# leggedrobotics/wild_visual_navigation

Hardware: NVIDIA H100
Metric: frames/sec end-to-end (DINO feat + seg + MLP train-step) at 448x448 (higher is better)
Workload: dtype bf16 operands / fp32 accumulate (ViT, STEGO head, per-pixel MLP); fp32 (k-means, train step)

## Files before the change

wild_visual_navigation_b200/csrc/common.cuh:

```cuda
#pragma once

#include <cuda.h>
#include <cuda_bf16.h>
#include <cuda_runtime.h>
#include <stdint.h>
#include <stdio.h>

namespace wvn {

__device__ __forceinline__ uint32_t smem_u32(const void* p) {
  return static_cast<uint32_t>(__cvta_generic_to_shared(p));
}

__device__ __forceinline__ bool elect_one_sync() {
  uint32_t pred;
  asm volatile(
      "{\n\t"
      ".reg .pred p;\n\t"
      "elect.sync _|p, 0xffffffff;\n\t"
      "selp.u32 %0, 1, 0, p;\n\t"
      "}"
      : "=r"(pred));
  return pred != 0;
}

__device__ __forceinline__ uint32_t pack_bf16x2(float lo, float hi) {
  __nv_bfloat162 v = __floats2bfloat162_rn(lo, hi);
  return *reinterpret_cast<uint32_t*>(&v);
}

__device__ __forceinline__ float bf16_lo(uint32_t v) { return __uint_as_float(v << 16); }
__device__ __forceinline__ float bf16_hi(uint32_t v) { return __uint_as_float(v & 0xffff0000u); }

__device__ __forceinline__ void mbar_init(uint64_t* bar, uint32_t count) {
  asm volatile("mbarrier.init.shared::cta.b64 [%0], %1;" ::"r"(smem_u32(bar)), "r"(count) : "memory");
}

__device__ __forceinline__ void fence_mbar_init() {
  asm volatile("fence.mbarrier_init.release.cluster;" ::: "memory");
}

__device__ __forceinline__ void mbar_arrive_expect_tx(uint64_t* bar, uint32_t bytes) {
  asm volatile("mbarrier.arrive.expect_tx.shared::cta.b64 _, [%0], %1;" ::"r"(smem_u32(bar)), "r"(bytes)
               : "memory");
}

__device__ __forceinline__ void mbar_arrive(uint64_t* bar) {
  asm volatile("mbarrier.arrive.shared::cta.b64 _, [%0];" ::"r"(smem_u32(bar)) : "memory");
}

__device__ __forceinline__ bool mbar_try_wait(uint64_t* bar, uint32_t parity) {
  uint32_t ok;
  asm volatile(
      "{\n\t"
      ".reg .pred p;\n\t"
      "mbarrier.try_wait.parity.shared::cta.b64 p, [%1], %2;\n\t"
      "selp.u32 %0, 1, 0, p;\n\t"
      "}"
      : "=r"(ok)
      : "r"(smem_u32(bar)), "r"(parity)
      : "memory");
  return ok != 0;
}

__device__ __forceinline__ bool mbar_test_wait(uint64_t* bar, uint32_t parity) {
  uint32_t ok;
  asm volatile(
      "{\n\t"
      ".reg .pred p;\n\t"
      "mbarrier.test_wait.parity.shared::cta.b64 p, [%1], %2;\n\t"
      "selp.u32 %0, 1, 0, p;\n\t"
      "}"
      : "=r"(ok)
      : "r"(smem_u32(bar)), "r"(parity)
      : "memory");
  return ok != 0;
}

#ifndef WVN_MBAR_TIMEOUT_CYCLES
#define WVN_MBAR_TIMEOUT_CYCLES 4000000000ll
#endif

#ifndef WVN_MBAR_HINT_NS
#define WVN_MBAR_HINT_NS 0
#endif
#define WVN_STR2(x) #x
#define WVN_STR(x) WVN_STR2(x)
#if WVN_MBAR_HINT_NS > 0
#define WVN_TRY_WAIT_PTX "mbarrier.try_wait.parity.shared::cta.b64 p, [%1], %2, " WVN_STR(WVN_MBAR_HINT_NS) ";\n\t"
#else
#define WVN_TRY_WAIT_PTX "mbarrier.try_wait.parity.shared::cta.b64 p, [%1], %2;\n\t"
#endif

__device__ __forceinline__ bool mbar_try_wait_many(uint32_t bar_addr, uint32_t parity) {
  uint32_t ok;
  asm volatile(
      "{\n\t"
      ".reg .pred p;\n\t"
      ".reg .u32 n;\n\t"
      "mov.u32 n, 65536;\n\t"
      "WVN_WAIT_LOOP:\n\t"
      WVN_TRY_WAIT_PTX
      "@p bra WVN_WAIT_DONE;\n\t"
      "sub.u32 n, n, 1;\n\t"
      "setp.ne.u32 p, n, 0;\n\t"
      "@p bra WVN_WAIT_LOOP;\n\t"
      "WVN_WAIT_DONE:\n\t"
      "selp.u32 %0, 1, 0, p;\n\t"
      "}"
      : "=r"(ok)
      : "r"(bar_addr), "r"(parity)
      : "memory");
  return ok != 0;
}

__device__ __forceinline__ void mbar_wait(uint64_t* bar, uint32_t parity) {
  if (mbar_try_wait(bar, parity)) return;
  const uint32_t addr = smem_u32(bar);
  const long long t0 = clock64();
  while (!mbar_try_wait_many(addr, parity)) {
    if (clock64() - t0 > WVN_MBAR_TIMEOUT_CYCLES) {
#ifdef WVN_MBAR_DIAG
      printf("[wvn] mbarrier timeout: block (%d,%d) thread %d bar@%u parity %u\n", blockIdx.x, blockIdx.y,
             threadIdx.x, addr, parity);
#endif
      __trap();
    }
  }
}

__device__ __forceinline__ void fence_proxy_async_smem() {
  asm volatile("fence.proxy.async.shared::cta;" ::: "memory");
}

__device__ __forceinline__ void tma_load_2d(const CUtensorMap* map, uint64_t* bar, void* smem_dst, int32_t c0,
                                            int32_t c1) {
  asm volatile(
      "cp.async.bulk.tensor.2d.shared::cluster.global.mbarrier::complete_tx::bytes [%0], [%1, {%3, %4}], [%2];" ::"r"(
          smem_u32(smem_dst)),
      "l"(reinterpret_cast<uint64_t>(map)), "r"(smem_u32(bar)), "r"(c0), "r"(c1)
      : "memory");
}

__device__ __forceinline__ void tma_load_2d_mcast(const CUtensorMap* map, uint64_t* bar, void* smem_dst, int32_t c0,
                                                  int32_t c1, uint16_t cta_mask) {
  asm volatile(
      "cp.async.bulk.tensor.2d.shared::cluster.global.mbarrier::complete_tx::bytes.multicast::cluster"
      " [%0], [%1, {%4, %5}], [%2], %3;" ::"r"(smem_u32(smem_dst)),
      "l"(reinterpret_cast<uint64_t>(map)), "r"(smem_u32(bar)), "h"(cta_mask), "r"(c0), "r"(c1)
      : "memory");
}

__device__ __forceinline__ void tma_store_2d(const CUtensorMap* map, const void* smem_src, int32_t c0, int32_t c1) {
  asm volatile("cp.async.bulk.tensor.2d.global.shared::cta.bulk_group [%0, {%2, %3}], [%1];" ::"l"(
                   reinterpret_cast<uint64_t>(map)),
               "r"(smem_u32(smem_src)), "r"(c0), "r"(c1)
               : "memory");
}
__device__ __forceinline__ void tma_reduce_add_2d(const CUtensorMap* map, const void* smem_src, int32_t c0, int32_t c1) {
  asm volatile("cp.reduce.async.bulk.tensor.2d.global.shared::cta.add.bulk_group [%0, {%2, %3}], [%1];" ::"l"(
                   reinterpret_cast<uint64_t>(map)),
               "r"(smem_u32(smem_src)), "r"(c0), "r"(c1)
               : "memory");
}
__device__ __forceinline__ void tma_store_commit() { asm volatile("cp.async.bulk.commit_group;" ::: "memory"); }
template <int N>
__device__ __forceinline__ void tma_store_wait_read() {
  asm volatile("cp.async.bulk.wait_group.read %0;" ::"n"(N) : "memory");
}
template <int N>
__device__ __forceinline__ void tma_store_wait_all() {
  asm volatile("cp.async.bulk.wait_group %0;" ::"n"(N) : "memory");
}

__device__ __forceinline__ uint32_t cluster_ctarank() {
  uint32_t r;
  asm volatile("mov.u32 %0, %%cluster_ctarank;" : "=r"(r));
  return r;
}

__device__ __forceinline__ void cluster_sync_all() {
  asm volatile("barrier.cluster.arrive.release.aligned;" ::: "memory");
  asm volatile("barrier.cluster.wait.acquire.aligned;" ::: "memory");
}

__device__ __forceinline__ void tma_prefetch_desc(const CUtensorMap* map) {
  asm volatile("prefetch.tensormap [%0];" ::"l"(reinterpret_cast<uint64_t>(map)) : "memory");
}

__device__ __forceinline__ uint64_t make_sw128_kmajor_desc(uint32_t smem_addr) {
  uint64_t d = 0;
  d |= static_cast<uint64_t>((smem_addr & 0x3ffff) >> 4);
  d |= static_cast<uint64_t>(1) << 16;
  d |= static_cast<uint64_t>(1024 >> 4) << 32;
  d |= static_cast<uint64_t>(1) << 62;
  return d;
}

__device__ __forceinline__ void wgmma_fence() { asm volatile("wgmma.fence.sync.aligned;" ::: "memory"); }
__device__ __forceinline__ void wgmma_commit() { asm volatile("wgmma.commit_group.sync.aligned;" ::: "memory"); }
template <int N>
__device__ __forceinline__ void wgmma_wait() {
  asm volatile("wgmma.wait_group.sync.aligned %0;" ::"n"(N) : "memory");
}

template <int N>
__device__ __forceinline__ void wgmma_fence_regs(float (&d)[N]) {
#pragma unroll
  for (int i = 0; i < N; ++i) asm volatile("" : "+f"(d[i])::"memory");
}
template <int N>
__device__ __forceinline__ void wgmma_fence_regs(uint32_t (&a)[N]) {
#pragma unroll
  for (int i = 0; i < N; ++i) asm volatile("" : "+r"(a[i])::"memory");
}

template <int N>
__device__ __forceinline__ void setmaxnreg_inc() { asm volatile("setmaxnreg.inc.sync.aligned.u32 %0;" ::"n"(N)); }
template <int N>
__device__ __forceinline__ void setmaxnreg_dec() { asm volatile("setmaxnreg.dec.sync.aligned.u32 %0;" ::"n"(N)); }

__device__ __forceinline__ void wgmma_m64n32k16_ss(float (&d)[16], uint64_t desc_a, uint64_t desc_b, uint32_t accumulate) {
  asm volatile(
      "{\n\t"
      ".reg .pred p;\n\t"
      "setp.ne.b32 p, %18, 0;\n\t"
      "wgmma.mma_async.sync.aligned.m64n32k16.f32.bf16.bf16 "
      "{%0, %1, %2, %3, %4, %5, %6, %7, %8, %9, %10, %11, %12, %13, %14, %15}, "
      "%16, %17, p, 1, 1, 0, 0;\n\t"
      "}"
      : "+f"(d[0]), "+f"(d[1]), "+f"(d[2]), "+f"(d[3]), "+f"(d[4]), "+f"(d[5]), "+f"(d[6]), "+f"(d[7]),
        "+f"(d[8]), "+f"(d[9]), "+f"(d[10]), "+f"(d[11]), "+f"(d[12]), "+f"(d[13]), "+f"(d[14]), "+f"(d[15])
      : "l"(desc_a), "l"(desc_b), "r"(accumulate));
}

__device__ __forceinline__ void wgmma_m64n64k16_ss(float (&d)[32], uint64_t desc_a, uint64_t desc_b, uint32_t accumulate) {
  asm volatile(
      "{\n\t"
      ".reg .pred p;\n\t"
      "setp.ne.b32 p, %34, 0;\n\t"
      "wgmma.mma_async.sync.aligned.m64n64k16.f32.bf16.bf16 "
      "{%0, %1, %2, %3, %4, %5, %6, %7, %8, %9, %10, %11, %12, %13, %14, %15, %16, %17, %18, %19, %20, "
      "%21, %22, %23, %24, %25, %26, %27, %28, %29, %30, %31}, "
      "%32, %33, p, 1, 1, 0, 0;\n\t"
      "}"
      : "+f"(d[0]), "+f"(d[1]), "+f"(d[2]), "+f"(d[3]), "+f"(d[4]), "+f"(d[5]), "+f"(d[6]), "+f"(d[7]),
        "+f"(d[8]), "+f"(d[9]), "+f"(d[10]), "+f"(d[11]), "+f"(d[12]), "+f"(d[13]), "+f"(d[14]), "+f"(d[15]),
        "+f"(d[16]), "+f"(d[17]), "+f"(d[18]), "+f"(d[19]), "+f"(d[20]), "+f"(d[21]), "+f"(d[22]), "+f"(d[23]),
        "+f"(d[24]), "+f"(d[25]), "+f"(d[26]), "+f"(d[27]), "+f"(d[28]), "+f"(d[29]), "+f"(d[30]), "+f"(d[31])
      : "l"(desc_a), "l"(desc_b), "r"(accumulate));
}

__device__ __forceinline__ void wgmma_m64n128k16_ss(float (&d)[64], uint64_t desc_a, uint64_t desc_b, uint32_t accumulate) {
  asm volatile(
      "{\n\t"
      ".reg .pred p;\n\t"
      "setp.ne.b32 p, %66, 0;\n\t"
      "wgmma.mma_async.sync.aligned.m64n128k16.f32.bf16.bf16 "
      "{%0, %1, %2, %3, %4, %5, %6, %7, %8, %9, %10, %11, %12, %13, %14, %15, %16, %17, %18, %19, %20, "
      "%21, %22, %23, %24, %25, %26, %27, %28, %29, %30, %31, %32, %33, %34, %35, %36, %37, %38, %39, "
      "%40, %41, %42, %43, %44, %45, %46, %47, %48, %49, %50, %51, %52, %53, %54, %55, %56, %57, %58, "
      "%59, %60, %61, %62, %63}, "
      "%64, %65, p, 1, 1, 0, 0;\n\t"
      "}"
      : "+f"(d[0]), "+f"(d[1]), "+f"(d[2]), "+f"(d[3]), "+f"(d[4]), "+f"(d[5]), "+f"(d[6]), "+f"(d[7]),
        "+f"(d[8]), "+f"(d[9]), "+f"(d[10]), "+f"(d[11]), "+f"(d[12]), "+f"(d[13]), "+f"(d[14]), "+f"(d[15]),
        "+f"(d[16]), "+f"(d[17]), "+f"(d[18]), "+f"(d[19]), "+f"(d[20]), "+f"(d[21]), "+f"(d[22]), "+f"(d[23]),
        "+f"(d[24]), "+f"(d[25]), "+f"(d[26]), "+f"(d[27]), "+f"(d[28]), "+f"(d[29]), "+f"(d[30]), "+f"(d[31]),
        "+f"(d[32]), "+f"(d[33]), "+f"(d[34]), "+f"(d[35]), "+f"(d[36]), "+f"(d[37]), "+f"(d[38]), "+f"(d[39]),
        "+f"(d[40]), "+f"(d[41]), "+f"(d[42]), "+f"(d[43]), "+f"(d[44]), "+f"(d[45]), "+f"(d[46]), "+f"(d[47]),
        "+f"(d[48]), "+f"(d[49]), "+f"(d[50]), "+f"(d[51]), "+f"(d[52]), "+f"(d[53]), "+f"(d[54]), "+f"(d[55]),
        "+f"(d[56]), "+f"(d[57]), "+f"(d[58]), "+f"(d[59]), "+f"(d[60]), "+f"(d[61]), "+f"(d[62]), "+f"(d[63])
      : "l"(desc_a), "l"(desc_b), "r"(accumulate));
}

__device__ __forceinline__ void wgmma_m64n64k16_rs(float (&d)[32], uint32_t a0, uint32_t a1, uint32_t a2, uint32_t a3,
                                                   uint64_t desc_b, uint32_t accumulate) {
  asm volatile(
      "{\n\t"
      ".reg .pred p;\n\t"
      "setp.ne.b32 p, %37, 0;\n\t"
      "wgmma.mma_async.sync.aligned.m64n64k16.f32.bf16.bf16 "
      "{%0, %1, %2, %3, %4, %5, %6, %7, %8, %9, %10, %11, %12, %13, %14, %15, %16, %17, %18, %19, %20, "
      "%21, %22, %23, %24, %25, %26, %27, %28, %29, %30, %31}, "
      "{%32, %33, %34, %35}, %36, p, 1, 1, 0;\n\t"
      "}"
      : "+f"(d[0]), "+f"(d[1]), "+f"(d[2]), "+f"(d[3]), "+f"(d[4]), "+f"(d[5]), "+f"(d[6]), "+f"(d[7]),
        "+f"(d[8]), "+f"(d[9]), "+f"(d[10]), "+f"(d[11]), "+f"(d[12]), "+f"(d[13]), "+f"(d[14]), "+f"(d[15]),
        "+f"(d[16]), "+f"(d[17]), "+f"(d[18]), "+f"(d[19]), "+f"(d[20]), "+f"(d[21]), "+f"(d[22]), "+f"(d[23]),
        "+f"(d[24]), "+f"(d[25]), "+f"(d[26]), "+f"(d[27]), "+f"(d[28]), "+f"(d[29]), "+f"(d[30]), "+f"(d[31])
      : "r"(a0), "r"(a1), "r"(a2), "r"(a3), "l"(desc_b), "r"(accumulate));
}

__device__ __forceinline__ void named_bar_sync(int id, int nthreads) {
  asm volatile("bar.sync %0, %1;" ::"r"(id), "r"(nthreads) : "memory");
}
__device__ __forceinline__ void named_bar_arrive(int id, int nthreads) {
  asm volatile("bar.arrive %0, %1;" ::"r"(id), "r"(nthreads) : "memory");
}

__device__ __forceinline__ void sts128(uint32_t addr, uint32_t a, uint32_t b, uint32_t c, uint32_t d) {
  asm volatile("st.shared.v4.b32 [%0], {%1, %2, %3, %4};" ::"r"(addr), "r"(a), "r"(b), "r"(c), "r"(d) : "memory");
}
__device__ __forceinline__ uint4 lds128(uint32_t addr) {
  uint4 v;
  asm volatile("ld.shared.v4.b32 {%0, %1, %2, %3}, [%4];" : "=r"(v.x), "=r"(v.y), "=r"(v.z), "=r"(v.w) : "r"(addr) : "memory");
  return v;
}

__device__ __forceinline__ void st_global_v4(void* p, uint32_t a, uint32_t b, uint32_t c, uint32_t d) {
  asm volatile("st.global.v4.b32 [%0], {%1, %2, %3, %4};" ::"l"(p), "r"(a), "r"(b), "r"(c), "r"(d) : "memory");
}

__device__ __forceinline__ float warp_sum(float v) {
#pragma unroll
  for (int o = 16; o > 0; o >>= 1) v += __shfl_xor_sync(0xffffffffu, v, o);
  return v;
}

__device__ __forceinline__ float warp_max(float v) {
#pragma unroll
  for (int o = 16; o > 0; o >>= 1) v = fmaxf(v, __shfl_xor_sync(0xffffffffu, v, o));
  return v;
}

}
```

wild_visual_navigation_b200/csrc/gemm_wgmma.cu:

```cuda
#include <stdlib.h>

#include <algorithm>

#include "common.cuh"
#include "gemm.h"
#include "host_common.h"

namespace wvn {

namespace {

constexpr int BM = 128;
constexpr int BK = 64;
constexpr int kConsumerWarps = 8;
constexpr int kNumThreads = 128 + kConsumerWarps * 32;
constexpr int kMaxSmemBytes = 227 * 1024;
constexpr int kMaxStages = 8;
constexpr int kFixedSmemBytes = 1024  + 1024 ;

template <bool ROW_OWNER>
struct TileIter {
  int num_m, num_n, m_blk, n_blk, lin;
  __device__ TileIter(int nm, int nn) : num_m(nm), num_n(nn), m_blk(0), n_blk(0), lin(0) {
    if (ROW_OWNER) { m_blk = blockIdx.x; n_blk = 0; }
    else { lin = blockIdx.x; m_blk = lin / num_n; n_blk = lin % num_n; }
  }
  __device__ bool valid() const { return m_blk < num_m; }
  __device__ void next() {
    if (ROW_OWNER) { if (++n_blk == num_n) { n_blk = 0; m_blk += gridDim.x; } }
    else { lin += gridDim.x; m_blk = lin / num_n; n_blk = lin % num_n; }
  }
};

template <int BN>
struct GemmCfg {
  static constexpr uint32_t kABytes = BM * BK * 2;
  static constexpr uint32_t kBBytes = BN * BK * 2;
  static constexpr uint32_t kStageBytes = kABytes + kBBytes;
  static constexpr int kStagesRaw = (kMaxSmemBytes - kFixedSmemBytes) / kStageBytes;
  static constexpr int kStages = kStagesRaw > kMaxStages ? kMaxStages : kStagesRaw;
  static constexpr uint32_t kSmemBytes = kStages * kStageBytes + kFixedSmemBytes;
  static constexpr int kN128 = BN / 128;
  static constexpr int kN64 = (BN % 128) / 64;
  static constexpr int kN32 = (BN % 64) / 32;
};

__device__ __forceinline__ float gelu_erf_fast(float x) {
  const float t = fminf(fabsf(x), 5.5f);
  float p = fmaf(-0.0003865310864f, t, 0.006509808358f);
  p = fmaf(p, t, -0.05048002675f);
  p = fmaf(p, t, -0.4613505006f);
  p = fmaf(p, t, -1.150225043f);
  p = fmaf(p, t, -1.00010848f);
  float e;
  asm("ex2.approx.ftz.f32 %0, %1;" : "=f"(e) : "f"(p));
  return fmaf(-t, e, fmaxf(x, 0.f));
}

template <int EPI, int ACT, int NREG>
__device__ __forceinline__ void epilogue_frag(const GemmArgs& args, const float (&d)[NREG], const int row0,
                                              const int col_base, const int lane, float (&head_partial)[2]) {
  const int q = lane & 3;
  bool ok[2];
  long long orow[2];
  int frame[2], tok[2];
#pragma unroll
  for (int h = 0; h < 2; ++h) {
    const int row = row0 + 8 * h;
    ok[h] = row < args.M;
    orow[h] = row;
    frame[h] = tok[h] = 0;
    if (EPI == EPI_PATCH) {
      frame[h] = row / args.tokens_in;
      tok[h] = row - frame[h] * args.tokens_in;
      orow[h] = static_cast<long long>(frame[h]) * args.npad + 1 + tok[h];
    } else if (EPI == EPI_QKV) {
      frame[h] = row / args.npad;
      tok[h] = row - frame[h] * args.npad;
    }
  }
#pragma unroll
  for (int j = 0; j < NREG / 4; ++j) {
    const int col = col_base + 8 * j + 2 * q;
    float2 b = make_float2(0.f, 0.f);
    if (args.bias != nullptr) b = __ldg(reinterpret_cast<const float2*>(args.bias + col));
#pragma unroll
    for (int h = 0; h < 2; ++h) {
      float v0 = d[4 * j + 2 * h] + b.x, v1 = d[4 * j + 2 * h + 1] + b.y;
      if (ACT == ACT_RELU) {
        v0 = fmaxf(v0, 0.f);
        v1 = fmaxf(v1, 0.f);
      } else if (ACT == ACT_GELU) {
        v0 = gelu_erf_fast(v0);
        v1 = gelu_erf_fast(v1);
      }
      if (!ok[h]) continue;
      if (EPI == EPI_BF16) {
        *reinterpret_cast<uint32_t*>(reinterpret_cast<__nv_bfloat16*>(args.out) + orow[h] * args.ldo + col) = pack_bf16x2(v0, v1);
      } else if (EPI == EPI_F32) {
        *reinterpret_cast<float2*>(reinterpret_cast<float*>(args.out) + orow[h] * args.ldo + col) = make_float2(v0, v1);
      } else if (EPI == EPI_RESID_F32) {
        asm volatile("red.global.add.v2.f32 [%0], {%1, %2};" ::"l"(reinterpret_cast<float*>(args.out) + orow[h] * args.ldo + col),
                     "f"(v0), "f"(v1)
                     : "memory");
      } else if (EPI == EPI_PATCH) {
        const float2 pe = __ldg(reinterpret_cast<const float2*>(args.pos + static_cast<long long>(1 + tok[h]) * args.ldo + col));
        *reinterpret_cast<float2*>(reinterpret_cast<float*>(args.out) + orow[h] * args.ldo + col) = make_float2(v0 + pe.x, v1 + pe.y);
      } else if (EPI == EPI_QKV) {
        const int which = col / args.dim;
        const int within = col - which * args.dim;
        const long long bh = static_cast<long long>(frame[h]) * args.heads + (within >> 6);
        if (which < 2) {
          __nv_bfloat16* base = reinterpret_cast<__nv_bfloat16*>(which == 0 ? args.q : args.k);
          *reinterpret_cast<uint32_t*>(base + (bh * args.npad + tok[h]) * 64 + (within & 63)) = pack_bf16x2(v0, v1);
        } else {
          __nv_bfloat16* dst = reinterpret_cast<__nv_bfloat16*>(args.vt) + (bh * 64 + (within & 63)) * args.npad + tok[h];
          dst[0] = __float2bfloat16_rn(v0);
          dst[args.npad] = __float2bfloat16_rn(v1);
        }
      } else if (EPI == EPI_MLP_HEAD) {
        if (col < args.feat) {
          const uint32_t xv = __ldg(reinterpret_cast<const uint32_t*>(
              reinterpret_cast<const __nv_bfloat16*>(args.x) + orow[h] * args.ldx + col));
          const float d0 = v0 - bf16_lo(xv), d1 = v1 - bf16_hi(xv);
          head_partial[h] = fmaf(d0, d0, head_partial[h]);
          if (col + 1 < args.feat) head_partial[h] = fmaf(d1, d1, head_partial[h]);
        } else if (col == args.trav_col) {
          args.trav[orow[h]] = 1.f / (1.f + __expf(-v0));
        }
      }
    }
  }
}

template <int BN, int EPI, int ACT>
__global__ void __launch_bounds__(kNumThreads, 1)
gemm_bf16_kernel(const __grid_constant__ CUtensorMap tmap_a, const __grid_constant__ CUtensorMap tmap_b,
                 const GemmArgs args) {
  using Cfg = GemmCfg<BN>;
  constexpr int STAGES = Cfg::kStages;

  extern __shared__ uint8_t smem_raw[];
  uint8_t* smem = reinterpret_cast<uint8_t*>((reinterpret_cast<uintptr_t>(smem_raw) + 1023) & ~uintptr_t(1023));
  uint8_t* smem_b = smem;
  uint8_t* smem_a = smem + STAGES * Cfg::kBBytes;
  uint64_t* bars = reinterpret_cast<uint64_t*>(smem_a + STAGES * Cfg::kABytes);
  uint64_t* full_bar = bars;
  uint64_t* empty_bar = bars + kMaxStages;

  const int warp = threadIdx.x >> 5;
  const int lane = threadIdx.x & 31;

  const int num_m = (args.M + BM - 1) / BM;
  const int num_n = args.N / BN;
  const int num_k = args.K / BK;
  constexpr bool ROW_OWNER = (EPI == EPI_MLP_HEAD);

  if (threadIdx.x == 0) {
    tma_prefetch_desc(&tmap_a);
    tma_prefetch_desc(&tmap_b);
    for (int i = 0; i < kMaxStages; ++i) {
      mbar_init(&full_bar[i], 1);
      mbar_init(&empty_bar[i], kConsumerWarps);
    }
    fence_mbar_init();
  }
  __syncthreads();

  if (warp < 4) {
    setmaxnreg_dec<40>();
    if (warp == 0) {
      int stage = 0;
      uint32_t phase = 0;
      for (TileIter<ROW_OWNER> it(num_m, num_n); it.valid(); it.next()) {
        const int m_eff = args.reverse_m ? num_m - 1 - it.m_blk : it.m_blk;
        for (int kb = 0; kb < num_k; ++kb) {
          mbar_wait(&empty_bar[stage], phase ^ 1);
          if (elect_one_sync()) {
            mbar_arrive_expect_tx(&full_bar[stage], Cfg::kStageBytes);
            tma_load_2d(&tmap_a, &full_bar[stage], smem_a + stage * Cfg::kABytes, kb * BK, m_eff * BM);
            tma_load_2d(&tmap_b, &full_bar[stage], smem_b + stage * Cfg::kBBytes, kb * BK, it.n_blk * BN);
          }
          __syncwarp();
          if (++stage == STAGES) { stage = 0; phase ^= 1; }
        }
      }
    }
  } else {
    setmaxnreg_inc<232>();
    const int cwarp = warp - 4;
    const int wg = cwarp >> 2;
    const int row_in_tile = wg * 64 + (cwarp & 3) * 16 + (lane >> 2);
    float acc128[Cfg::kN128 > 0 ? Cfg::kN128 : 1][64];
    float acc64[32];
    float acc32[16];
    float head_partial[2] = {0.f, 0.f};
    int stage = 0;
    uint32_t phase = 0;
    for (TileIter<ROW_OWNER> it(num_m, num_n); it.valid(); it.next()) {
      int prev_stage = 0;
      for (int kb = 0; kb < num_k; ++kb) {
        mbar_wait(&full_bar[stage], phase);
        const uint64_t desc_a = make_sw128_kmajor_desc(smem_u32(smem_a + stage * Cfg::kABytes + wg * 64 * 128));
        const uint32_t b_addr = smem_u32(smem_b + stage * Cfg::kBBytes);
#pragma unroll
        for (int c = 0; c < Cfg::kN128; ++c) wgmma_fence_regs(acc128[c]);
        if (Cfg::kN64) wgmma_fence_regs(acc64);
        if (Cfg::kN32) wgmma_fence_regs(acc32);
        wgmma_fence();
#pragma unroll
        for (int k = 0; k < BK / 16; ++k) {
          const uint32_t accumulate = (kb | k) != 0 ? 1u : 0u;
#pragma unroll
          for (int c = 0; c < Cfg::kN128; ++c)
            wgmma_m64n128k16_ss(acc128[c], desc_a + 2 * k, make_sw128_kmajor_desc(b_addr + c * 128 * 128) + 2 * k, accumulate);
          if (Cfg::kN64)
            wgmma_m64n64k16_ss(acc64, desc_a + 2 * k, make_sw128_kmajor_desc(b_addr + Cfg::kN128 * 128 * 128) + 2 * k, accumulate);
          if (Cfg::kN32)
            wgmma_m64n32k16_ss(acc32, desc_a + 2 * k,
                               make_sw128_kmajor_desc(b_addr + (Cfg::kN128 * 128 + Cfg::kN64 * 64) * 128) + 2 * k, accumulate);
        }
        wgmma_commit();
        if (kb > 0) {
          wgmma_wait<1>();
          if (lane == 0) mbar_arrive(&empty_bar[prev_stage]);
        }
        prev_stage = stage;
        if (++stage == STAGES) { stage = 0; phase ^= 1; }
      }
      wgmma_wait<0>();
#pragma unroll
      for (int c = 0; c < Cfg::kN128; ++c) wgmma_fence_regs(acc128[c]);
      if (Cfg::kN64) wgmma_fence_regs(acc64);
      if (Cfg::kN32) wgmma_fence_regs(acc32);
      if (lane == 0) mbar_arrive(&empty_bar[prev_stage]);

      const int m_eff = args.reverse_m ? num_m - 1 - it.m_blk : it.m_blk;
      const int row0 = m_eff * BM + row_in_tile;
      const int col0 = it.n_blk * BN;
#pragma unroll
      for (int c = 0; c < Cfg::kN128; ++c)
        epilogue_frag<EPI, ACT>(args, acc128[c], row0, col0 + c * 128, lane, head_partial);
      if (Cfg::kN64) epilogue_frag<EPI, ACT>(args, acc64, row0, col0 + Cfg::kN128 * 128, lane, head_partial);
      if (Cfg::kN32) epilogue_frag<EPI, ACT>(args, acc32, row0, col0 + Cfg::kN128 * 128 + Cfg::kN64 * 64, lane, head_partial);

      if (EPI == EPI_MLP_HEAD && it.n_blk == num_n - 1) {
#pragma unroll
        for (int h = 0; h < 2; ++h) {
          float s = head_partial[h];
          s += __shfl_xor_sync(0xffffffffu, s, 1);
          s += __shfl_xor_sync(0xffffffffu, s, 2);
          head_partial[h] = 0.f;
          const int row = row0 + 8 * h;
          if ((lane & 3) == 0 && row < args.M) {
            const float loss = s / static_cast<float>(args.feat);
            const float mean = __ldg(args.cg_mean), sd = __ldg(args.cg_std);
            const float shifted = mean + sd * args.cg_std_factor;
            const float lo = fmaxf(shifted - sd, 0.f);
            const float hi = shifted + sd;
            const float xc = fminf(fmaxf(loss, lo), hi);
            args.conf[row] = 1.f - (xc - lo) / (hi - lo);
            if (args.loss_reco != nullptr) args.loss_reco[row] = loss;
          }
        }
      }
    }
  }
}

template <int BN, int EPI, int ACT>
int launch_gemm(const GemmArgs& a, const CUtensorMap& ta, const CUtensorMap& tb, cudaStream_t stream) {
  using Cfg = GemmCfg<BN>;
  static_assert(Cfg::kStages >= 2, "tile too wide for the shared-memory budget");
  auto kern = gemm_bf16_kernel<BN, EPI, ACT>;
  static bool attr_set = false;
  if (!attr_set) {
    WVN_CHECK_CUDA(cudaFuncSetAttribute(kern, cudaFuncAttributeMaxDynamicSharedMemorySize, kMaxSmemBytes));
    attr_set = true;
  }
  const int num_m = (a.M + BM - 1) / BM, num_n = a.N / BN;
  const int num_tiles = (EPI == EPI_MLP_HEAD) ? num_m : num_m * num_n;
  int grid = sm_count();
  if (a.max_ctas > 0 && a.max_ctas < grid) grid = a.max_ctas;
  if (grid > num_tiles) grid = num_tiles;
  prof_begin(PROF_GEMM, stream);
  kern<<<grid, kNumThreads, Cfg::kSmemBytes, stream>>>(ta, tb, a);
  prof_end(PROF_GEMM, stream);
  WVN_CHECK_LAUNCH("gemm_bf16_kernel");
  return WVN_OK;
}

template <int BN>
int dispatch_epi(const GemmArgs& a, const CUtensorMap& ta, const CUtensorMap& tb, cudaStream_t s) {
  switch (a.epi) {
    case EPI_BF16:
      if (a.act == ACT_NONE) return launch_gemm<BN, EPI_BF16, ACT_NONE>(a, ta, tb, s);
      if (a.act == ACT_RELU) return launch_gemm<BN, EPI_BF16, ACT_RELU>(a, ta, tb, s);
      if (a.act == ACT_GELU) return launch_gemm<BN, EPI_BF16, ACT_GELU>(a, ta, tb, s);
      break;
    case EPI_F32:
      if (a.act == ACT_NONE) return launch_gemm<BN, EPI_F32, ACT_NONE>(a, ta, tb, s);
      break;
    case EPI_RESID_F32:
      if (a.act == ACT_NONE) return launch_gemm<BN, EPI_RESID_F32, ACT_NONE>(a, ta, tb, s);
      break;
    case EPI_PATCH:
      if (a.act == ACT_NONE) return launch_gemm<BN, EPI_PATCH, ACT_NONE>(a, ta, tb, s);
      break;
    case EPI_QKV:
      if (a.act == ACT_NONE) return launch_gemm<BN, EPI_QKV, ACT_NONE>(a, ta, tb, s);
      break;
    case EPI_MLP_HEAD:
      if (a.act == ACT_NONE) return launch_gemm<BN, EPI_MLP_HEAD, ACT_NONE>(a, ta, tb, s);
      break;
  }
  return set_error(WVN_ERR_INVALID, "gemm: unsupported epilogue/activation combination (%d, %d)", a.epi, a.act);
}

}

int pick_block_n(int N) {
  if (N % 256 == 0) return 256;
  if (N % 224 == 0) return 224;
  if (N % 192 == 0) return 192;
  if (N % 128 == 0) return 128;
  if (N % 64 == 0) return 64;
  return 0;
}

int gemm_bf16(const GemmArgs& a, const void* A, long long lda, const void* W, int block_n, cudaStream_t stream) {
  WVN_REQUIRE(a.M > 0 && a.N > 0 && a.K > 0, "gemm: empty problem (M=%d N=%d K=%d)", a.M, a.N, a.K);
  WVN_REQUIRE(a.K % BK == 0, "gemm: K=%d must be a multiple of %d (pad the operands)", a.K, BK);
  if (block_n == 0) block_n = pick_block_n(a.N);
  WVN_REQUIRE(block_n == 64 || block_n == 128 || block_n == 192 || block_n == 224 || block_n == 256,
              "gemm: bad block_n %d", block_n);
  WVN_REQUIRE(a.N % block_n == 0, "gemm: N=%d must be a multiple of block_n=%d (pad the weights)", a.N, block_n);
  if (a.epi == EPI_MLP_HEAD)
    WVN_REQUIRE(a.feat > 0 && a.trav_col % 32 == 0 && a.trav_col >= a.feat && a.trav_col < a.N && a.x != nullptr &&
                    a.trav != nullptr && a.conf != nullptr && a.cg_mean != nullptr && a.cg_std != nullptr &&
                    a.ldx % 8 == 0 && a.ldx >= a.trav_col,
                "gemm: bad MLP-head epilogue arguments (feat=%d trav_col=%d N=%d)", a.feat, a.trav_col, a.N);
  if (a.epi == EPI_QKV)
    WVN_REQUIRE(a.dim % 64 == 0 && a.N == 3 * a.dim && a.heads * 64 == a.dim && a.npad % 8 == 0,
                "gemm: bad QKV epilogue geometry (dim=%d heads=%d npad=%d N=%d)", a.dim, a.heads, a.npad, a.N);
  if (a.epi == EPI_F32 || a.epi == EPI_RESID_F32) WVN_REQUIRE(a.ldo % 4 == 0, "gemm: fp32 output pitch must be a multiple of 4");
  if (a.epi == EPI_BF16) WVN_REQUIRE(a.ldo % 8 == 0, "gemm: bf16 output pitch must be a multiple of 8");
  CUtensorMap ta, tb;
  WVN_PROPAGATE(make_tmap_bf16_2d(&ta, A, a.K, a.M, static_cast<uint64_t>(lda) * 2, BK, BM));
  WVN_PROPAGATE(make_tmap_bf16_2d(&tb, W, a.K, a.N, static_cast<uint64_t>(a.K) * 2, BK, block_n));
  switch (block_n) {
    case 64: return dispatch_epi<64>(a, ta, tb, stream);
    case 128: return dispatch_epi<128>(a, ta, tb, stream);
    case 192: return dispatch_epi<192>(a, ta, tb, stream);
    case 224: return dispatch_epi<224>(a, ta, tb, stream);
    case 256: return dispatch_epi<256>(a, ta, tb, stream);
  }
  return set_error(WVN_ERR_INVALID, "gemm: unreachable");
}

}
```

Measured before the change: 839.4.

## Ping-pong consumer warpgroups on 64-row tiles with TMA-staged epilogue stores

Shrinks the GEMM M-tile to 64 rows and gives alternate tiles to the two consumer warpgroups, which take turns on the tensor cores through named barriers. One warpgroup can run its epilogue while the other runs its MMAs. Epilogue writes for bf16, fp32, residual-add and QKV outputs now go through swizzled shared-memory slices and are sent with TMA store or reduce-add, including a transposed V layout. This costs staging shared memory and so fewer pipeline stages, adds barrier complexity, and requires npad to be a multiple of the tile height for QKV.

Result: faster. 961.8 (median of 6 runs) (+14.6%).

```diff
diff --git a/wild_visual_navigation_b200/csrc/common.cuh b/wild_visual_navigation_b200/csrc/common.cuh
--- a/wild_visual_navigation_b200/csrc/common.cuh
+++ b/wild_visual_navigation_b200/csrc/common.cuh
@@ -151,16 +151,16 @@
       : "memory");
 }
 
-__device__ __forceinline__ void tma_store_2d(const CUtensorMap* map, const void* smem_src, int32_t c0, int32_t c1) {
+__device__ __forceinline__ void tma_store_2d(const CUtensorMap* map, uint32_t smem_src, int32_t c0, int32_t c1) {
   asm volatile("cp.async.bulk.tensor.2d.global.shared::cta.bulk_group [%0, {%2, %3}], [%1];" ::"l"(
                    reinterpret_cast<uint64_t>(map)),
-               "r"(smem_u32(smem_src)), "r"(c0), "r"(c1)
+               "r"(smem_src), "r"(c0), "r"(c1)
                : "memory");
 }
-__device__ __forceinline__ void tma_reduce_add_2d(const CUtensorMap* map, const void* smem_src, int32_t c0, int32_t c1) {
+__device__ __forceinline__ void tma_reduce_add_2d(const CUtensorMap* map, uint32_t smem_src, int32_t c0, int32_t c1) {
   asm volatile("cp.reduce.async.bulk.tensor.2d.global.shared::cta.add.bulk_group [%0, {%2, %3}], [%1];" ::"l"(
                    reinterpret_cast<uint64_t>(map)),
-               "r"(smem_u32(smem_src)), "r"(c0), "r"(c1)
+               "r"(smem_src), "r"(c0), "r"(c1)
                : "memory");
 }
 __device__ __forceinline__ void tma_store_commit() { asm volatile("cp.async.bulk.commit_group;" ::: "memory"); }
@@ -302,6 +302,15 @@
 __device__ __forceinline__ void sts128(uint32_t addr, uint32_t a, uint32_t b, uint32_t c, uint32_t d) {
   asm volatile("st.shared.v4.b32 [%0], {%1, %2, %3, %4};" ::"r"(addr), "r"(a), "r"(b), "r"(c), "r"(d) : "memory");
 }
+__device__ __forceinline__ void sts64(uint32_t addr, float a, float b) {
+  asm volatile("st.shared.v2.f32 [%0], {%1, %2};" ::"r"(addr), "f"(a), "f"(b) : "memory");
+}
+__device__ __forceinline__ void sts32(uint32_t addr, uint32_t a) {
+  asm volatile("st.shared.b32 [%0], %1;" ::"r"(addr), "r"(a) : "memory");
+}
+__device__ __forceinline__ void sts16(uint32_t addr, __nv_bfloat16 a) {
+  asm volatile("st.shared.b16 [%0], %1;" ::"r"(addr), "h"(__bfloat16_as_ushort(a)) : "memory");
+}
 __device__ __forceinline__ uint4 lds128(uint32_t addr) {
   uint4 v;
   asm volatile("ld.shared.v4.b32 {%0, %1, %2, %3}, [%4];" : "=r"(v.x), "=r"(v.y), "=r"(v.z), "=r"(v.w) : "r"(addr) : "memory");
diff --git a/wild_visual_navigation_b200/csrc/gemm_wgmma.cu b/wild_visual_navigation_b200/csrc/gemm_wgmma.cu
--- a/wild_visual_navigation_b200/csrc/gemm_wgmma.cu
+++ b/wild_visual_navigation_b200/csrc/gemm_wgmma.cu
@@ -10,13 +10,14 @@
 
 namespace {
 
-constexpr int BM = 128;
+constexpr int BM = 64;
 constexpr int BK = 64;
 constexpr int kConsumerWarps = 8;
 constexpr int kNumThreads = 128 + kConsumerWarps * 32;
 constexpr int kMaxSmemBytes = 227 * 1024;
 constexpr int kMaxStages = 8;
 constexpr int kFixedSmemBytes = 1024  + 1024 ;
+constexpr int kSliceCols = 32;
 
 template <bool ROW_OWNER>
 struct TileIter {
@@ -32,14 +33,19 @@
   }
 };
 
-template <int BN>
+template <int EPI>
+constexpr bool kStaged = EPI == EPI_BF16 || EPI == EPI_F32 || EPI == EPI_RESID_F32 || EPI == EPI_QKV;
+
+template <int BN, int EPI>
 struct GemmCfg {
   static constexpr uint32_t kABytes = BM * BK * 2;
   static constexpr uint32_t kBBytes = BN * BK * 2;
   static constexpr uint32_t kStageBytes = kABytes + kBBytes;
-  static constexpr int kStagesRaw = (kMaxSmemBytes - kFixedSmemBytes) / kStageBytes;
+  static constexpr uint32_t kSliceBytes = BM * kSliceCols * ((EPI == EPI_F32 || EPI == EPI_RESID_F32) ? 4 : 2);
+  static constexpr uint32_t kStagingBytes = kStaged<EPI> ? 2 * 2 * kSliceBytes : 0;
+  static constexpr int kStagesRaw = (kMaxSmemBytes - kFixedSmemBytes - kStagingBytes) / kStageBytes;
   static constexpr int kStages = kStagesRaw > kMaxStages ? kMaxStages : kStagesRaw;
-  static constexpr uint32_t kSmemBytes = kStages * kStageBytes + kFixedSmemBytes;
+  static constexpr uint32_t kSmemBytes = kStages * kStageBytes + kStagingBytes + kFixedSmemBytes;
   static constexpr int kN128 = BN / 128;
   static constexpr int kN64 = (BN % 128) / 64;
   static constexpr int kN32 = (BN % 64) / 32;
@@ -57,26 +63,30 @@
   return fmaf(-t, e, fmaxf(x, 0.f));
 }
 
+template <int ACT>
+__device__ __forceinline__ float activate(float v) {
+  if (ACT == ACT_RELU) return fmaxf(v, 0.f);
+  if (ACT == ACT_GELU) return gelu_erf_fast(v);
+  return v;
+}
+
 template <int EPI, int ACT, int NREG>
 __device__ __forceinline__ void epilogue_frag(const GemmArgs& args, const float (&d)[NREG], const int row0,
                                               const int col_base, const int lane, float (&head_partial)[2]) {
   const int q = lane & 3;
   bool ok[2];
   long long orow[2];
-  int frame[2], tok[2];
+  int tok[2];
 #pragma unroll
   for (int h = 0; h < 2; ++h) {
     const int row = row0 + 8 * h;
     ok[h] = row < args.M;
     orow[h] = row;
-    frame[h] = tok[h] = 0;
+    tok[h] = 0;
     if (EPI == EPI_PATCH) {
-      frame[h] = row / args.tokens_in;
-      tok[h] = row - frame[h] * args.tokens_in;
-      orow[h] = static_cast<long long>(frame[h]) * args.npad + 1 + tok[h];
-    } else if (EPI == EPI_QKV) {
-      frame[h] = row / args.npad;
-      tok[h] = row - frame[h] * args.npad;
+      const int frame = row / args.tokens_in;
+      tok[h] = row - frame * args.tokens_in;
+      orow[h] = static_cast<long long>(frame) * args.npad + 1 + tok[h];
     }
   }
 #pragma unroll
@@ -86,38 +96,11 @@
     if (args.bias != nullptr) b = __ldg(reinterpret_cast<const float2*>(args.bias + col));
 #pragma unroll
     for (int h = 0; h < 2; ++h) {
-      float v0 = d[4 * j + 2 * h] + b.x, v1 = d[4 * j + 2 * h + 1] + b.y;
-      if (ACT == ACT_RELU) {
-        v0 = fmaxf(v0, 0.f);
-        v1 = fmaxf(v1, 0.f);
-      } else if (ACT == ACT_GELU) {
-        v0 = gelu_erf_fast(v0);
-        v1 = gelu_erf_fast(v1);
-      }
+      const float v0 = activate<ACT>(d[4 * j + 2 * h] + b.x), v1 = activate<ACT>(d[4 * j + 2 * h + 1] + b.y);
       if (!ok[h]) continue;
-      if (EPI == EPI_BF16) {
-        *reinterpret_cast<uint32_t*>(reinterpret_cast<__nv_bfloat16*>(args.out) + orow[h] * args.ldo + col) = pack_bf16x2(v0, v1);
-      } else if (EPI == EPI_F32) {
-        *reinterpret_cast<float2*>(reinterpret_cast<float*>(args.out) + orow[h] * args.ldo + col) = make_float2(v0, v1);
-      } else if (EPI == EPI_RESID_F32) {
-        asm volatile("red.global.add.v2.f32 [%0], {%1, %2};" ::"l"(reinterpret_cast<float*>(args.out) + orow[h] * args.ldo + col),
-                     "f"(v0), "f"(v1)
-                     : "memory");
-      } else if (EPI == EPI_PATCH) {
+      if (EPI == EPI_PATCH) {
         const float2 pe = __ldg(reinterpret_cast<const float2*>(args.pos + static_cast<long long>(1 + tok[h]) * args.ldo + col));
         *reinterpret_cast<float2*>(reinterpret_cast<float*>(args.out) + orow[h] * args.ldo + col) = make_float2(v0 + pe.x, v1 + pe.y);
-      } else if (EPI == EPI_QKV) {
-        const int which = col / args.dim;
-        const int within = col - which * args.dim;
-        const long long bh = static_cast<long long>(frame[h]) * args.heads + (within >> 6);
-        if (which < 2) {
-          __nv_bfloat16* base = reinterpret_cast<__nv_bfloat16*>(which == 0 ? args.q : args.k);
-          *reinterpret_cast<uint32_t*>(base + (bh * args.npad + tok[h]) * 64 + (within & 63)) = pack_bf16x2(v0, v1);
-        } else {
-          __nv_bfloat16* dst = reinterpret_cast<__nv_bfloat16*>(args.vt) + (bh * 64 + (within & 63)) * args.npad + tok[h];
-          dst[0] = __float2bfloat16_rn(v0);
-          dst[args.npad] = __float2bfloat16_rn(v1);
-        }
       } else if (EPI == EPI_MLP_HEAD) {
         if (col < args.feat) {
           const uint32_t xv = __ldg(reinterpret_cast<const uint32_t*>(
@@ -133,18 +116,83 @@
   }
 }
 
+template <int EPI, int ACT, int NREG>
+__device__ __forceinline__ void store_frag(const GemmArgs& args, const CUtensorMap* tm0, const CUtensorMap* tm1,
+                                           const CUtensorMap* tm2, const float (&d)[NREG], const int row_tile,
+                                           const int col_base, const int row_local, const int lane, const bool leader,
+                                           const int bar_id, const uint32_t staging, const uint32_t slice_bytes,
+                                           const int slice0) {
+  const int q = lane & 3;
+#pragma unroll
+  for (int s = 0; s < NREG / 16; ++s) {
+    const int col = col_base + kSliceCols * s;
+    const int si = slice0 + s;
+    const uint32_t buf = staging + (si & 1) * slice_bytes;
+    int which = 0, within = 0;
+    if (EPI == EPI_QKV) {
+      which = col / args.dim;
+      within = col - which * args.dim;
+    }
+    if (leader) {
+      if (si == 0) tma_store_wait_read<0>();
+      else tma_store_wait_read<1>();
+    }
+    named_bar_sync(bar_id, 128);
+#pragma unroll
+    for (int js = 0; js < 4; ++js) {
+      const int j = 4 * s + js;
+      const int c = col + 8 * js + 2 * q;
+      float2 b = make_float2(0.f, 0.f);
+      if (args.bias != nullptr) b = __ldg(reinterpret_cast<const float2*>(args.bias + c));
+#pragma unroll
+      for (int h = 0; h < 2; ++h) {
+        const float v0 = activate<ACT>(d[4 * j + 2 * h] + b.x), v1 = activate<ACT>(d[4 * j + 2 * h + 1] + b.y);
+        const int r = row_local + 8 * h;
+        if (EPI == EPI_F32 || EPI == EPI_RESID_F32) {
+          sts64(buf + r * 128 + ((((2 * js + (q >> 1)) ^ (r & 7))) << 4) + (q & 1) * 8, v0, v1);
+        } else if (EPI == EPI_QKV && which == 2) {
+          const int dd = 8 * js + 2 * q;
+          const uint32_t t = 2 * r;
+          sts16(buf + dd * 128 + (((t >> 4) ^ (dd & 7)) << 4) + (t & 15), __float2bfloat16_rn(v0));
+          sts16(buf + (dd + 1) * 128 + (((t >> 4) ^ ((dd + 1) & 7)) << 4) + (t & 15), __float2bfloat16_rn(v1));
+        } else {
+          sts32(buf + r * 64 + ((js ^ ((r >> 1) & 3)) << 4) + q * 4, pack_bf16x2(v0, v1));
+        }
+      }
+    }
+    fence_proxy_async_smem();
+    named_bar_sync(bar_id, 128);
+    if (leader) {
+      if (EPI == EPI_BF16 || EPI == EPI_F32) {
+        tma_store_2d(tm0, buf, col, row_tile);
+      } else if (EPI == EPI_RESID_F32) {
+        tma_reduce_add_2d(tm0, buf, col, row_tile);
+      } else if (EPI == EPI_QKV) {
+        const int frame = row_tile / args.npad;
+        const int tok0 = row_tile - frame * args.npad;
+        const int bh = frame * args.heads + (within >> 6);
+        if (which < 2) tma_store_2d(which == 0 ? tm0 : tm1, buf, within & 63, bh * args.npad + tok0);
+        else tma_store_2d(tm2, buf, tok0, bh * 64 + (within & 63));
+      }
+      tma_store_commit();
+    }
+  }
+}
+
 template <int BN, int EPI, int ACT>
 __global__ void __launch_bounds__(kNumThreads, 1)
 gemm_bf16_kernel(const __grid_constant__ CUtensorMap tmap_a, const __grid_constant__ CUtensorMap tmap_b,
-                 const GemmArgs args) {
-  using Cfg = GemmCfg<BN>;
+                 const __grid_constant__ CUtensorMap tmap_c0, const __grid_constant__ CUtensorMap tmap_c1,
+                 const __grid_constant__ CUtensorMap tmap_c2, const GemmArgs args) {
+  using Cfg = GemmCfg<BN, EPI>;
   constexpr int STAGES = Cfg::kStages;
 
   extern __shared__ uint8_t smem_raw[];
   uint8_t* smem = reinterpret_cast<uint8_t*>((reinterpret_cast<uintptr_t>(smem_raw) + 1023) & ~uintptr_t(1023));
   uint8_t* smem_b = smem;
   uint8_t* smem_a = smem + STAGES * Cfg::kBBytes;
-  uint64_t* bars = reinterpret_cast<uint64_t*>(smem_a + STAGES * Cfg::kABytes);
+  uint8_t* smem_c = smem_a + STAGES * Cfg::kABytes;
+  uint64_t* bars = reinterpret_cast<uint64_t*>(smem_c + Cfg::kStagingBytes);
   uint64_t* full_bar = bars;
   uint64_t* empty_bar = bars + kMaxStages;
 
@@ -161,7 +209,7 @@
     tma_prefetch_desc(&tmap_b);
     for (int i = 0; i < kMaxStages; ++i) {
       mbar_init(&full_bar[i], 1);
-      mbar_init(&empty_bar[i], kConsumerWarps);
+      mbar_init(&empty_bar[i], kConsumerWarps / 2);
     }
     fence_mbar_init();
   }
@@ -190,18 +238,37 @@
     setmaxnreg_inc<232>();
     const int cwarp = warp - 4;
     const int wg = cwarp >> 2;
-    const int row_in_tile = wg * 64 + (cwarp & 3) * 16 + (lane >> 2);
+    const int row_local = (cwarp & 3) * 16 + (lane >> 2);
+    const bool leader = (threadIdx.x & 127) == 0;
+    const uint32_t staging = smem_u32(smem_c) + wg * 2 * Cfg::kSliceBytes;
+    if (kStaged<EPI> && leader) {
+      tma_prefetch_desc(&tmap_c0);
+      if (EPI == EPI_QKV) {
+        tma_prefetch_desc(&tmap_c1);
+        tma_prefetch_desc(&tmap_c2);
+      }
+    }
+    if (wg == 1) named_bar_arrive(1, 256);
     float acc128[Cfg::kN128 > 0 ? Cfg::kN128 : 1][64];
     float acc64[32];
     float acc32[16];
     float head_partial[2] = {0.f, 0.f};
     int stage = 0;
     uint32_t phase = 0;
+    int unit = 0;
     for (TileIter<ROW_OWNER> it(num_m, num_n); it.valid(); it.next()) {
+      const bool unit_end = !ROW_OWNER || it.n_blk == num_n - 1;
+      if ((unit & 1) != wg) {
+        for (int kb = 0; kb < num_k; ++kb)
+          if (++stage == STAGES) { stage = 0; phase ^= 1; }
+        if (unit_end) ++unit;
+        continue;
+      }
+      if (!ROW_OWNER || it.n_blk == 0) named_bar_sync(1 + wg, 256);
       int prev_stage = 0;
       for (int kb = 0; kb < num_k; ++kb) {
         mbar_wait(&full_bar[stage], phase);
-        const uint64_t desc_a = make_sw128_kmajor_desc(smem_u32(smem_a + stage * Cfg::kABytes + wg * 64 * 128));
+        const uint64_t desc_a = make_sw128_kmajor_desc(smem_u32(smem_a + stage * Cfg::kABytes));
         const uint32_t b_addr = smem_u32(smem_b + stage * Cfg::kBBytes);
 #pragma unroll
         for (int c = 0; c < Cfg::kN128; ++c) wgmma_fence_regs(acc128[c]);
@@ -228,6 +295,8 @@
         prev_stage = stage;
         if (++stage == STAGES) { stage = 0; phase ^= 1; }
       }
+      if (unit_end && (ROW_OWNER ? it.m_blk + static_cast<int>(gridDim.x) < num_m : it.lin + static_cast<int>(gridDim.x) < num_m * num_n))
+        named_bar_arrive(2 - wg, 256);
       wgmma_wait<0>();
 #pragma unroll
       for (int c = 0; c < Cfg::kN128; ++c) wgmma_fence_regs(acc128[c]);
@@ -236,13 +305,28 @@
       if (lane == 0) mbar_arrive(&empty_bar[prev_stage]);
 
       const int m_eff = args.reverse_m ? num_m - 1 - it.m_blk : it.m_blk;
-      const int row0 = m_eff * BM + row_in_tile;
+      const int row_tile = m_eff * BM;
       const int col0 = it.n_blk * BN;
-#pragma unroll
-      for (int c = 0; c < Cfg::kN128; ++c)
-        epilogue_frag<EPI, ACT>(args, acc128[c], row0, col0 + c * 128, lane, head_partial);
-      if (Cfg::kN64) epilogue_frag<EPI, ACT>(args, acc64, row0, col0 + Cfg::kN128 * 128, lane, head_partial);
-      if (Cfg::kN32) epilogue_frag<EPI, ACT>(args, acc32, row0, col0 + Cfg::kN128 * 128 + Cfg::kN64 * 64, lane, head_partial);
+      if (kStaged<EPI>) {
+        const int bar_id = 3 + wg;
+#pragma unroll
+        for (int c = 0; c < Cfg::kN128; ++c)
+          store_frag<EPI, ACT>(args, &tmap_c0, &tmap_c1, &tmap_c2, acc128[c], row_tile, col0 + c * 128, row_local, lane,
+                               leader, bar_id, staging, Cfg::kSliceBytes, 4 * c);
+        if (Cfg::kN64)
+          store_frag<EPI, ACT>(args, &tmap_c0, &tmap_c1, &tmap_c2, acc64, row_tile, col0 + Cfg::kN128 * 128, row_local,
+                               lane, leader, bar_id, staging, Cfg::kSliceBytes, 4 * Cfg::kN128);
+        if (Cfg::kN32)
+          store_frag<EPI, ACT>(args, &tmap_c0, &tmap_c1, &tmap_c2, acc32, row_tile, col0 + Cfg::kN128 * 128 + Cfg::kN64 * 64,
+                               row_local, lane, leader, bar_id, staging, Cfg::kSliceBytes, 4 * Cfg::kN128 + 2 * Cfg::kN64);
+      } else {
+        const int row0 = row_tile + row_local;
+#pragma unroll
+        for (int c = 0; c < Cfg::kN128; ++c)
+          epilogue_frag<EPI, ACT>(args, acc128[c], row0, col0 + c * 128, lane, head_partial);
+        if (Cfg::kN64) epilogue_frag<EPI, ACT>(args, acc64, row0, col0 + Cfg::kN128 * 128, lane, head_partial);
+        if (Cfg::kN32) epilogue_frag<EPI, ACT>(args, acc32, row0, col0 + Cfg::kN128 * 128 + Cfg::kN64 * 64, lane, head_partial);
+      }
 
       if (EPI == EPI_MLP_HEAD && it.n_blk == num_n - 1) {
 #pragma unroll
@@ -251,7 +335,7 @@
           s += __shfl_xor_sync(0xffffffffu, s, 1);
           s += __shfl_xor_sync(0xffffffffu, s, 2);
           head_partial[h] = 0.f;
-          const int row = row0 + 8 * h;
+          const int row = row_tile + row_local + 8 * h;
           if ((lane & 3) == 0 && row < args.M) {
             const float loss = s / static_cast<float>(args.feat);
             const float mean = __ldg(args.cg_mean), sd = __ldg(args.cg_std);
@@ -264,13 +348,16 @@
           }
         }
       }
-    }
+      if (unit_end) ++unit;
+    }
+    if (kStaged<EPI> && leader) tma_store_wait_all<0>();
   }
 }
 
 template <int BN, int EPI, int ACT>
-int launch_gemm(const GemmArgs& a, const CUtensorMap& ta, const CUtensorMap& tb, cudaStream_t stream) {
-  using Cfg = GemmCfg<BN>;
+int launch_gemm(const GemmArgs& a, const CUtensorMap& ta, const CUtensorMap& tb, const CUtensorMap (&tc)[3],
+                cudaStream_t stream) {
+  using Cfg = GemmCfg<BN, EPI>;
   static_assert(Cfg::kStages >= 2, "tile too wide for the shared-memory budget");
   auto kern = gemm_bf16_kernel<BN, EPI, ACT>;
   static bool attr_set = false;
@@ -284,34 +371,35 @@
   if (a.max_ctas > 0 && a.max_ctas < grid) grid = a.max_ctas;
   if (grid > num_tiles) grid = num_tiles;
   prof_begin(PROF_GEMM, stream);
-  kern<<<grid, kNumThreads, Cfg::kSmemBytes, stream>>>(ta, tb, a);
+  kern<<<grid, kNumThreads, Cfg::kSmemBytes, stream>>>(ta, tb, tc[0], tc[1], tc[2], a);
   prof_end(PROF_GEMM, stream);
   WVN_CHECK_LAUNCH("gemm_bf16_kernel");
   return WVN_OK;
 }
 
 template <int BN>
-int dispatch_epi(const GemmArgs& a, const CUtensorMap& ta, const CUtensorMap& tb, cudaStream_t s) {
+int dispatch_epi(const GemmArgs& a, const CUtensorMap& ta, const CUtensorMap& tb, const CUtensorMap (&tc)[3],
+                 cudaStream_t s) {
   switch (a.epi) {
     case EPI_BF16:
-      if (a.act == ACT_NONE) return launch_gemm<BN, EPI_BF16, ACT_NONE>(a, ta, tb, s);
-      if (a.act == ACT_RELU) return launch_gemm<BN, EPI_BF16, ACT_RELU>(a, ta, tb, s);
-      if (a.act == ACT_GELU) return launch_gemm<BN, EPI_BF16, ACT_GELU>(a, ta, tb, s);
+      if (a.act == ACT_NONE) return launch_gemm<BN, EPI_BF16, ACT_NONE>(a, ta, tb, tc, s);
+      if (a.act == ACT_RELU) return launch_gemm<BN, EPI_BF16, ACT_RELU>(a, ta, tb, tc, s);
+      if (a.act == ACT_GELU) return launch_gemm<BN, EPI_BF16, ACT_GELU>(a, ta, tb, tc, s);
       break;
     case EPI_F32:
-      if (a.act == ACT_NONE) return launch_gemm<BN, EPI_F32, ACT_NONE>(a, ta, tb, s);
+      if (a.act == ACT_NONE) return launch_gemm<BN, EPI_F32, ACT_NONE>(a, ta, tb, tc, s);
       break;
     case EPI_RESID_F32:
-      if (a.act == ACT_NONE) return launch_gemm<BN, EPI_RESID_F32, ACT_NONE>(a, ta, tb, s);
+      if (a.act == ACT_NONE) return launch_gemm<BN, EPI_RESID_F32, ACT_NONE>(a, ta, tb, tc, s);
       break;
     case EPI_PATCH:
-      if (a.act == ACT_NONE) return launch_gemm<BN, EPI_PATCH, ACT_NONE>(a, ta, tb, s);
+      if (a.act == ACT_NONE) return launch_gemm<BN, EPI_PATCH, ACT_NONE>(a, ta, tb, tc, s);
       break;
     case EPI_QKV:
-      if (a.act == ACT_NONE) return launch_gemm<BN, EPI_QKV, ACT_NONE>(a, ta, tb, s);
+      if (a.act == ACT_NONE) return launch_gemm<BN, EPI_QKV, ACT_NONE>(a, ta, tb, tc, s);
       break;
     case EPI_MLP_HEAD:
-      if (a.act == ACT_NONE) return launch_gemm<BN, EPI_MLP_HEAD, ACT_NONE>(a, ta, tb, s);
+      if (a.act == ACT_NONE) return launch_gemm<BN, EPI_MLP_HEAD, ACT_NONE>(a, ta, tb, tc, s);
       break;
   }
   return set_error(WVN_ERR_INVALID, "gemm: unsupported epilogue/activation combination (%d, %d)", a.epi, a.act);
@@ -341,19 +429,30 @@
                     a.ldx % 8 == 0 && a.ldx >= a.trav_col,
                 "gemm: bad MLP-head epilogue arguments (feat=%d trav_col=%d N=%d)", a.feat, a.trav_col, a.N);
   if (a.epi == EPI_QKV)
-    WVN_REQUIRE(a.dim % 64 == 0 && a.N == 3 * a.dim && a.heads * 64 == a.dim && a.npad % 8 == 0,
-                "gemm: bad QKV epilogue geometry (dim=%d heads=%d npad=%d N=%d)", a.dim, a.heads, a.npad, a.N);
+    WVN_REQUIRE(a.dim % 64 == 0 && a.N == 3 * a.dim && a.heads * 64 == a.dim && a.npad % 8 == 0 && a.npad % BM == 0 &&
+                    a.M % a.npad == 0,
+                "gemm: bad QKV epilogue geometry (dim=%d heads=%d npad=%d N=%d M=%d)", a.dim, a.heads, a.npad, a.N, a.M);
   if (a.epi == EPI_F32 || a.epi == EPI_RESID_F32) WVN_REQUIRE(a.ldo % 4 == 0, "gemm: fp32 output pitch must be a multiple of 4");
   if (a.epi == EPI_BF16) WVN_REQUIRE(a.ldo % 8 == 0, "gemm: bf16 output pitch must be a multiple of 8");
-  CUtensorMap ta, tb;
+  CUtensorMap ta, tb, tc[3] = {};
   WVN_PROPAGATE(make_tmap_bf16_2d(&ta, A, a.K, a.M, static_cast<uint64_t>(lda) * 2, BK, BM));
   WVN_PROPAGATE(make_tmap_bf16_2d(&tb, W, a.K, a.N, static_cast<uint64_t>(a.K) * 2, BK, block_n));
+  if (a.epi == EPI_BF16)
+    WVN_PROPAGATE(make_tmap_2d(&tc[0], a.out, 2, a.N, a.M, static_cast<uint64_t>(a.ldo) * 2, kSliceCols, BM, 64));
+  if (a.epi == EPI_F32 || a.epi == EPI_RESID_F32)
+    WVN_PROPAGATE(make_tmap_2d(&tc[0], a.out, 4, a.N, a.M, static_cast<uint64_t>(a.ldo) * 4, kSliceCols, BM, 128));
+  if (a.epi == EPI_QKV) {
+    const uint64_t bh = static_cast<uint64_t>(a.M / a.npad) * a.heads;
+    WVN_PROPAGATE(make_tmap_2d(&tc[0], a.q, 2, 64, bh * a.npad, 128, kSliceCols, BM, 64));
+    WVN_PROPAGATE(make_tmap_2d(&tc[1], a.k, 2, 64, bh * a.npad, 128, kSliceCols, BM, 64));
+    WVN_PROPAGATE(make_tmap_2d(&tc[2], a.vt, 2, a.npad, bh * 64, static_cast<uint64_t>(a.npad) * 2, BM, kSliceCols, 128));
+  }
   switch (block_n) {
-    case 64: return dispatch_epi<64>(a, ta, tb, stream);
-    case 128: return dispatch_epi<128>(a, ta, tb, stream);
-    case 192: return dispatch_epi<192>(a, ta, tb, stream);
-    case 224: return dispatch_epi<224>(a, ta, tb, stream);
-    case 256: return dispatch_epi<256>(a, ta, tb, stream);
+    case 64: return dispatch_epi<64>(a, ta, tb, tc, stream);
+    case 128: return dispatch_epi<128>(a, ta, tb, tc, stream);
+    case 192: return dispatch_epi<192>(a, ta, tb, tc, stream);
+    case 224: return dispatch_epi<224>(a, ta, tb, tc, stream);
+    case 256: return dispatch_epi<256>(a, ta, tb, tc, stream);
   }
   return set_error(WVN_ERR_INVALID, "gemm: unreachable");
 }
```
